# gardner-lab/syllable-detector-swift

Measured on AMD Instinct MI355X. Metric: audio frames/sec (256-pt STFT + 2-layer MLP), whole job, higher is better.
Workload: dtype f32 (I/O and accumulate; products as f16 hi/lo split x3 on MFMA)

## Files before the change

### syllable_detector_swift_amd/csrc/fused_plan.cpp

```cpp

#include <algorithm>
#include <cmath>
#include <cstdlib>
#include <cstring>

#include "fused_plan.hpp"

namespace sd {

namespace {

uint16_t to_half(float f)
{
    uint32_t x;
    std::memcpy(&x, &f, 4);
    const uint32_t sign = (x >> 16) & 0x8000u;
    const int32_t exp = (int32_t)((x >> 23) & 0xff) - 127 + 15;
    uint32_t man = x & 0x7fffffu;
    if (((x >> 23) & 0xff) == 0xff) return (uint16_t)(sign | 0x7c00u | (man ? 0x200u : 0));
    if (exp >= 31) return (uint16_t)(sign | 0x7c00u);
    if (exp <= 0) {
        if (exp < -10) return (uint16_t)sign;
        man |= 0x800000u;
        const int shift = 14 - exp;
        uint32_t h = man >> shift;
        const uint32_t rem = man & ((1u << shift) - 1), halfway = 1u << (shift - 1);
        if (rem > halfway || (rem == halfway && (h & 1))) h++;
        return (uint16_t)(sign | h);
    }
    uint32_t h = ((uint32_t)exp << 10) | (man >> 13);
    const uint32_t rem = man & 0x1fffu;
    if (rem > 0x1000u || (rem == 0x1000u && (h & 1))) h++;
    return (uint16_t)(sign | h);
}

float from_half(uint16_t h)
{
    const uint32_t sign = (uint32_t)(h & 0x8000u) << 16;
    const uint32_t exp = (h >> 10) & 0x1f, man = h & 0x3ffu;
// ... 148 lines not shown
        if (padp > W / 2) padp = 0;
#ifdef SYLDET_PLAN_NOPAD
        padp = 0;
#endif
        int chunk_bytes = 1024 + (padp ? 16 * (256 / padp) : 0);
        auto ring_chunks = [&](int waves) { return std::min(30, (160 * 1024 / waves - (row_bytes + 15) / 16 * 16) / chunk_bytes - 1); };
        auto fits = [&](int rc) { return rc >= (span + 255) / 256 + 1 && kFusedSTileFrames * hop <= rc * 256; };
        if (padp && !fits(ring_chunks(kFusedSBlock / 64))) {
            padp = 0;
            chunk_bytes = 1024;
        }
        const int s_waves = (!wide_band && (HQ == 1 || (HQ == 2 && fits(ring_chunks(kFusedSBlock / 64))))) ? kFusedSBlock / 64 : kFusedSBlock / 128;
        const int per_wave = 160 * 1024 / s_waves;
        const int RC = ring_chunks(s_waves);
        if (sym && H <= 16 && c.n_layers == 2 && fits(RC)) {
            d.s_ok = 1;
            d.s_waves = s_waves;
            d.s_padp = (padp && s_waves == kFusedSBlock / 64) ? padp : 0;
            d.s_perm = (hop / 4 + (d.s_padp ? hop / d.s_padp : 0)) % 2 == 1 ? 1 : 0;
#ifdef SYLDET_PLAN_NOPERM
            d.s_perm = (hop / 4) % 2 == 1 ? 1 : 0;
#endif
            d.s_ring_chunks = RC; d.s_pstride = PSs; d.s_tp = TP;
            d.s_lds_wave = per_wave;
            d.s_cs8 = 0;
            d.s_cs8_rc = 0;
            if (d.s_padp == 128 && hop == 128) {
                const int rc8 = std::min(16, (per_wave - (row_bytes + 15) / 16 * 16) / 1280);
                if (rc8 >= (span + 255) / 256 + 1) {
                    d.s_cs8 = 1;
                    d.s_cs8_rc = rc8;
                }
            }
            const int K2 = W / 64, c0 = W / 2;
            p.sfrag.assign((size_t)K2 * 2 * 2 * 2 * 64 * 8, 0);
            for (int ks = 0; ks < K2; ks++)
                for (int which = 0; which < 2; which++)
                    for (int m2 = 0; m2 < 2; m2++)
                        for (int l = 0; l < 64; l++)
                            for (int j = 0; j < 8; j++) {
                                const int r = 16 * m2 + (l & 15), m = 32 * ks + 8 * (l >> 4) + j;
                                double v = 0.0;
                                if (r < F) {
                                    const int k = g.f0 + r;
                                    const int kn = (int)(((int64_t)k * m) % N);
                                    const double ang = two_pi * (double)kn / (double)N;
                                    const double wm = 0.5 * ((double)win[(size_t)(c0 + m)] + (double)win[(size_t)(c0 - m)]);
                                    if (which == 0) {
                                        v = wm * std::cos(ang) * (m == 0 ? 0.5 : 1.0);
                                    } else if (m == 0) {
                                        const int kh = (int)(((int64_t)k * (W / 2)) % N);
                                        v = (double)win[0] * std::sin(two_pi * (double)kh / (double)N);
                                    } else {
                                        v = -wm * std::sin(ang);
                                    }
                                    if (which == 1 && k == 0) v = 0.0;
                                    v *= 8192.0;
                                }
                                uint16_t hi, lo;
                                split_half(v, hi, lo);
                                const size_t base = (((((size_t)ks * 2 + which) * 2 + m2) * 2) * 64 + l) * 8 + j;
                                p.sfrag[base] = hi;
                                p.sfrag[base + 64 * 8] = lo;
                            }
            p.slone.assign(64 * 8, 0.0f);
            for (int l = 0; l < 64; l++)
// ... 458 lines not shown
```

### syllable_detector_swift_amd/csrc/kernels.hpp

```cpp
#pragma once

#include <hip/hip_runtime.h>

#include <cstdint>

namespace sd {

constexpr int kMaxFns = 8;
constexpr int kMaxLayers = 8;

struct StftDesc {
    int N, W, M, logM;
    int hop, gap;
    int f0, F;
    int power_mode;
    const float *window;
    const float2 *tw;
    const float2 *sw;
    const int *row_of;
};

struct DevFn {
    int kind;
    int xoff, gain;
// ... 118 lines not shown
    int no_fold2;
    const uint4 *sfrag2;
    const float *swin2;
    const float *s2c;
    const uint4 *afrag_t2;
    const uint4 *afrag_w2;
    const uint4 *sfrag;
    const uint4 *afrag_w;
    const float *slone;
    const uint4 *dfrag;
    const uint4 *afrag;
    const uint4 *afrag_t;
    const int *koff;
    const float *bias0;
    const float *rvec;
    const float *w1, *b1;
    const float *out_params;
    const double *thresholds;
    float *spect_out;
    int spect_power;
    float guard_r;
    float guard_c;
    float guard_c_range;
    float guard_range_r;
    float guard_rel_r, guard_rel_c;
    int guard_se_abs_r, guard_se_abs_c;
    float guard_spect;
    int guard_se_abs_s;
    float guard_loud;
    FixList fix;
    int force_classic;
    int no_fold;
    int ko;
    unsigned long long *stamps;
};
struct FusedNet {
    const uint4 *afrag_t, *afrag_w, *afrag_t2, *afrag_w2;
    const float *bias0, *rvec, *w1, *b1, *out_params;
    const double *thresholds;
    float w_unscale, guard_r, guard_rel_r, guard_range_r, guard_loud;
    int guard_se_abs_r;
};
struct FusedMulti {
    const FusedNet *nets;
    const int *net_of;
    const int *row_of;
};

constexpr int kMlpxBlock = 512;
constexpr int kMlpxTile = 128;
struct MlpxDesc {
    int F, T, KB, H;
    int rule;
    int scaling;
    int col_stride;
    int p_stride;
    float w_unscale, b1, oa, og, ob;
    int lds_afrag, lds_colh, lds_coll, lds_p, lds_pq, lds_ss, lds_red, lds_total;
    const uint4 *afrag;
    const float *bias0, *w1;
    const double *thresholds;
};
constexpr int kBdftBlock = 512;
struct BdftDesc {
    int hop, kb0, f0;
    int R;
// ... 98 lines not shown
```

### syllable_detector_swift_amd/csrc/kernels_fused_s.hip

```cpp

#include "fused_common.hpp"

namespace sd {

namespace {

using namespace fused_dev;

constexpr int kTile = kFusedSTileFrames;

typedef __attribute__((address_space(3))) void lds_void;

__device__ __forceinline__ float rem_lo(float a, unsigned h)
{
    float r;
    asm("v_fma_mix_f32 %0, %1, 1.0, -%2 op_sel_hi:[0,0,1]" : "=v"(r) : "v"(a), "v"(h));
    return r;
}
__device__ __forceinline__ float rem_hi(float a, unsigned h)
{
    float r;
    asm("v_fma_mix_f32 %0, %1, 1.0, -%2 op_sel:[0,0,1] op_sel_hi:[0,0,1]" : "=v"(r) : "v"(a), "v"(h));
    return r;
}
__device__ __forceinline__ unsigned cvt_pk(float a, float b)
{
    unsigned r;
    asm("v_cvt_pk_f16_f32 %0, %1, %2" : "=v"(r) : "v"(a), "v"(b));
    return r;
}
__device__ __forceinline__ floatx4 s16x4(const int16_t *p)
{
    const uint2 v = *reinterpret_cast<const uint2 *>(p);
    constexpr float k = 1.0f / 32768.0f;
    return floatx4{(float)(int16_t)(v.x & 0xffffu) * k, (float)((int)v.x >> 16) * k, (float)(int16_t)(v.y & 0xffffu) * k,
                   (float)((int)v.y >> 16) * k};
}
__device__ __forceinline__ float s16x1(const int16_t *p) { return (float)p[0] * (1.0f / 32768.0f); }

__device__ __forceinline__ void split2(float a, float b, unsigned &hi, unsigned &lo)
{
    hi = cvt_pk(a, b);
    lo = cvt_pk(rem_lo(a, hi), rem_hi(b, hi));
}

template <int K2, bool GEN, int HQ, int NW, int PADP = 0, bool F2 = false, int NT = 1, bool SPECT = false, bool MN = false, bool S16 = false>
__global__ void __launch_bounds__(64 * NW, 1)
fused_s_kernel(const FusedDesc d, const float *__restrict__ samples, int64_t stride, int64_t s_eff, int64_t E,
               float *__restrict__ outputs, uint8_t *__restrict__ flags, const FusedNet *__restrict__ nets, const int *__restrict__ net_of,
               const int *__restrict__ row_of)
{
    static_assert(!(MN && SPECT), "the spectrogram instantiation runs no network");
    static_assert(!S16 || (K2 == 4 && F2 && PADP == 0 && NT == 1 && HQ == 1 && NW == 8 && !SPECT), "16-bit PCM: the twice-folded form on the plain ring");
    extern __shared__ __attribute__((aligned(16))) unsigned char smem[];
    const int tid = threadIdx.x;
    const int lane = tid & 63;
    const int wave = __builtin_amdgcn_readfirstlane(tid >> 6);
    const int n = lane & 15, g = lane >> 4;
    constexpr int kWaves = NW;
    const int c = blockIdx.y;
    const int T = d.T, H = d.H, hop = d.hop;
    constexpr int W = 64 * K2;
    const int n_out = GEN ? d.n_out : 1;
    const int64_t e_b = ((int64_t)blockIdx.x * kWaves + wave) * d.s_seg_evals;
    if (e_b >= E) return;
    const int64_t e_e = (e_b + d.s_seg_evals < E) ? e_b + d.s_seg_evals : E;
    const int seg_len = (int)(e_e - e_b);
    const int tiles = (seg_len + (T - 1) + kTile - 1) / kTile;
    const unsigned e_b32 = (unsigned)e_b;
    const FusedNet *nt = MN ? nets + __builtin_amdgcn_readfirstlane(net_of[c]) : nullptr;
#define SD_NET(f) (MN ? nt->f : d.f)

    const int fr = d.s_perm ? (n < 4 ? 2 * n : (n >= 12 ? 2 * (n - 8) : 2 * (n - 4) + 1)) : n;

    unsigned char *wbase = smem + (size_t)wave * d.s_lds_wave;
    const int RC = PADP == 1 ? d.s_cs8_rc : d.s_ring_chunks, R = RC * (S16 ? 512 : 256);
    constexpr bool CS8 = PADP == 1;
    static_assert(!CS8 || (F2 && HQ == 1 && NT == 1), "staggered chunks: the twice-folded form at hop 128");
    constexpr int kSub = PADP > 1 ? 256 / PADP : 1;
    constexpr int kChunkB = CS8 ? 1280 : 1024 + (PADP > 1 ? 16 * kSub : 0);
    auto sk = [](int i) { return PADP > 1 ? 4 * (i / (PADP > 1 ? PADP : 1)) : 0; };
    float *ring = reinterpret_cast<float *>(wbase);
    const int16_t *ring16 = reinterpret_cast<const int16_t *>(wbase);
    const int PS = d.s_pstride, TP = d.s_tp;
    float *rows = reinterpret_cast<float *>(wbase + (size_t)(RC + (CS8 ? 0 : 1)) * kChunkB);
    float *zquad = rows + (T - 1 + kTile) * PS;
    constexpr bool kTbl = HQ == 2 && NW == 8;
    float *gtab = zquad + 8 * HQ + 32 * g;
    {
        const int nz = ((T - 1 + kTile) * PS + 8 * HQ + 128) / 4;
        for (int i = lane; i < nz; i += 64) reinterpret_cast<floatx4 *>(rows)[i] = floatx4{0.f, 0.f, 0.f, 0.f};
    }

    constexpr int KB = F2 ? 1 : K2;
    half8 as_[KB][2][2], ad_[KB][2][2];
    if (!F2) {
#pragma unroll
        for (int ks = 0; ks < KB; ks++)
#pragma unroll
            for (int m = 0; m < 2; m++)
#pragma unroll
                for (int p = 0; p < 2; p++) {
                    as_[ks][m][p] = as_half8(reinterpret_cast<const uint32x4 *>(d.sfrag)[(((ks * 2 + 0) * 2 + m) * 2 + p) * 64 + lane]);
                    ad_[ks][m][p] = as_half8(reinterpret_cast<const uint32x4 *>(d.sfrag)[(((ks * 2 + 1) * 2 + m) * 2 + p) * 64 + lane]);
                }
    }
    half8 b2[F2 ? 2 : 1][F2 ? 4 * NT : 1][2];
    float w1c[F2 ? 16 : 1], w2c[F2 ? 16 : 1], ce[4 * NT], w192 = 0.0f;
#pragma unroll
// ... 38 lines not shown
    const int rc = MN ? bank_row(row_of, c) : c;
    const float *row = S16 ? reinterpret_cast<const float *>(reinterpret_cast<const int16_t *>(samples) + (int64_t)rc * stride)
                           : samples + (int64_t)rc * stride;
    const __amdgpu_buffer_rsrc_t in_rs = __builtin_amdgcn_make_buffer_rsrc(const_cast<float *>(row), 0, (int)(s_eff * (S16 ? 2 : 4)), 0x00020000);
    const __amdgpu_buffer_rsrc_t out_rs = __builtin_amdgcn_make_buffer_rsrc(
        outputs ? outputs + (int64_t)rc * E * n_out : nullptr, 0, outputs ? (int)(E * n_out * 4) : 0, 0x00020000);
    const __amdgpu_buffer_rsrc_t flg_rs = __builtin_amdgcn_make_buffer_rsrc(flags ? flags + (int64_t)rc * E : nullptr, 0, flags ? (int)E : 0, 0x00020000);
    const __amdgpu_buffer_rsrc_t spc_rs = __builtin_amdgcn_make_buffer_rsrc(
        SPECT ? d.spect_out + (int64_t)c * E * d.F : nullptr, 0, SPECT ? (int)(E * d.F * 4) : 0, 0x00020000);

    const unsigned org = (unsigned)((e_b * hop + d.gap) * (S16 ? 2 : 4));
    int cn = 0, slot = 0;
    auto issue_upto = [&](int last) {
        while (cn <= last) {
            const unsigned voff = org + (unsigned)cn * 1024u + (unsigned)lane * 16u;
            if (CS8) {
                const int pad = ((cn & 6) << 1) | (cn & 1);
                __builtin_amdgcn_raw_ptr_buffer_load_lds(in_rs, (lds_void *)(wbase + slot * kChunkB + 16 * pad), 16, voff, 0, 0, 2 );
            } else if (PADP == 0) {
                __builtin_amdgcn_raw_ptr_buffer_load_lds(in_rs, (lds_void *)(wbase + slot * 1024), 16, voff, 0, 0, 2 );
                if (slot == 0) __builtin_amdgcn_raw_ptr_buffer_load_lds(in_rs, (lds_void *)(wbase + RC * 1024), 16, voff, 0, 0, 2);
            } else {
#pragma unroll
                for (int k = 0; k < kSub; k++)
                    if (lane / (64 / kSub) == k) {
                        __builtin_amdgcn_raw_ptr_buffer_load_lds(in_rs, (lds_void *)(wbase + slot * kChunkB + 16 * k), 16, voff, 0, 0, 2);
                        if (slot == 0) __builtin_amdgcn_raw_ptr_buffer_load_lds(in_rs, (lds_void *)(wbase + RC * kChunkB + 16 * k), 16, voff, 0, 0, 2);
                    }
            }
            cn++;
            slot = slot + 1 == RC ? 0 : slot + 1;
        }
    };
    const int span = (kTile - 1) * hop + W;
    constexpr int kChunkLog = S16 ? 9 : 8;
    auto need = [&](int t) { return (kTile * hop * t + span - 1) >> kChunkLog; };
    auto allowed = [&](int t) { return RC - 1 + ((kTile * hop * t) >> kChunkLog); };

    unsigned fo = (unsigned)(hop * fr);
    unsigned sb1 = (unsigned)((fr >> 1) * kChunkB), sb2 = (unsigned)(((fr >> 1) + (fr & 1)) * kChunkB);
    const int jq1 = (fr >> 1) & 7, jq2 = ((fr >> 1) + (fr & 1)) & 7;
    const unsigned cb1 = (unsigned)(16 * (((jq1 & 6) << 1) | (jq1 & 1)) + ((fr & 1) ? 512 : 0));
    const unsigned cb2 = (unsigned)(16 * (((jq2 & 6) << 1) | (jq2 & 1)) + ((fr & 1) ? 0 : 512));
    float *prow = rows + (T - 1 + fr) * PS;
    const float *erow = rows + n * PS;
    const float *pv_p[3], *sv_p[3];
#pragma unroll
    for (int tt = 0; tt < 3; tt++) {
        const int t = g + 4 * tt;
        pv_p[tt] = t < T ? erow + t * PS + 4 * HQ * t : zquad;
        sv_p[tt] = t < T ? erow + t * PS + 4 * HQ * TP : zquad;
    }
    float *pt_p[3];
#pragma unroll
    for (int m = 0; m < 3; m++) pt_p[m] = 4 * m + g < TP ? prow + 4 * HQ * (4 * m + g) : zquad + 4 * HQ;

    const float c_b1 = GEN ? (g < n_out ? SD_NET(b1)[g] : 0.0f) : SD_NET(b1)[0];
    float lean_oa = 0.0f, lean_og = 1.0f, lean_ob = 0.0f;
    if (d.n_out_fns == 1) {
        const int o = (GEN && g < n_out) ? g : 0;
        lean_oa = SD_NET(out_params)[0]; lean_og = SD_NET(out_params)[1 + o]; lean_ob = SD_NET(out_params)[1 + n_out + o];
    }
    float b0g[HQ], w1g[HQ], w1o[4][HQ], rvg[HQ];
#pragma unroll
    for (int q = 0; q < HQ; q++) {
        const int u = 4 * q + g;
// ... 6 lines not shown
    if (kTbl && n == 0) {
#pragma unroll
        for (int q = 0; q < HQ; q++) {
            gtab[8 + q] = b0g[q];
            gtab[8 + HQ + q] = w1g[q];
            gtab[8 + 6 * HQ + q] = rvg[q];
#pragma unroll
            for (int o = 0; o < 4; o++) gtab[8 + 2 * HQ + o * HQ + q] = w1o[o][q];
        }
    }
    const bool multi = GEN && n_out > 1;
    const double thr_g = SD_NET(thresholds)[(GEN && g < n_out) ? g : 0];
    if (kTbl && n == 0) {
        gtab[22] = c_b1; gtab[23] = lean_oa; gtab[24] = lean_og; gtab[25] = lean_ob;
        *reinterpret_cast<double *>(gtab + 26) = thr_g;
    }
    const bool counts = !GEN || n_out == 1 ? true : (g < n_out && (g == 0 || d.rule == 1));
    const int tf0 = GEN ? d.tf0 : 0, tf1 = GEN ? d.tf1 : 2, norm = GEN ? d.norm : 1;
    const int scaling = GEN ? d.scaling : 0;
    const float klog = scaling == 1 ? 0.6931471805599453f : 6.020599913279624f;
    bool binv[8 * NT];
#pragma unroll
    for (int i = 0; i < 8 * NT; i++) {
        const int tau = i >> 3, ii = i & 7;
        binv[i] = (F2 ? 32 * tau + (ii < 4 ? 8 * g + d.s2_pe + 2 * ii : 8 * g + d.s2_po + 2 * (ii - 4)) : (ii < 4 ? 4 * g + ii : 16 + 4 * g + (ii - 4))) < d.F;
    }
    const float kmag = pow2f(-13 - d.col_shift);
    const bool guard_on = d.fix.counters != nullptr;
    const float guard_k = norm == 1 ? SD_NET(guard_r) : (norm == 0 ? SD_NET(guard_rel_r) : SD_NET(guard_range_r));
    const float mn_wu = MN ? nt->w_unscale : 0.0f, mn_loud = MN ? nt->guard_loud : 0.0f;
    const int mn_se_abs = MN ? nt->guard_se_abs_r : 0;
#undef SD_NET

    issue_upto(need(0) < allowed(0) ? need(0) : allowed(0));
    int se_ref = 0;

#ifdef SYLDET_S_STAMPS
    unsigned long long st_vm = 0, st_lg = 0;
    const unsigned long long st_begin = __builtin_amdgcn_s_memtime();
#define SD_STAMP(var, stmt) { asm volatile("s_waitcnt lgkmcnt(0)" ::: "memory"); const unsigned long long t0_ = __builtin_amdgcn_s_memtime(); stmt; \
                              const unsigned long long t1_ = __builtin_amdgcn_s_memtime(); var += t1_ - t0_; }
#else
#define SD_STAMP(var, stmt) { stmt; }
#endif
#ifndef SYLDET_S_NO_PREWAIT
    __builtin_amdgcn_s_waitcnt(0x0F70);
#endif
#if defined(SYLDET_S_SETPRIO_SECOND)
    if (wave >= kWaves / 2) __builtin_amdgcn_s_setprio(1);
#elif defined(SYLDET_S_SETPRIO_FIRST)
    if (wave < kWaves / 2) __builtin_amdgcn_s_setprio(1);
#endif
    for (int t = 0; t < tiles; t++) {
        SD_STAMP(st_vm, if (t == 0) asm volatile("s_waitcnt vmcnt(0)" ::: "memory"); else if (SPECT) asm volatile("s_waitcnt vmcnt(5)" ::: "memory");
                        else asm volatile("s_waitcnt vmcnt(2)" ::: "memory"));
        const float *f1 = reinterpret_cast<const float *>(wbase + sb1 + cb1);
        const float *f2 = reinterpret_cast<const float *>(wbase + sb2 + cb2);
        const float *fp = CS8 ? f1 : ring + fo + sk((int)fo);

        floatx4 P1[2][2], P3[2][2], P2[2][2], P4[2][2];
        float P2w[2], P4w[2], x64 = 0.0f, x192 = 0.0f;
        if (F2) {
#pragma unroll
            for (int ks = 0; ks < 2; ks++) {
                if (CS8) {
                    const float *a1 = f1 + 32 * ks + 8 * g, *a2 = f2 + 32 * ks + 8 * g;
                    const float *b1 = f1 + 120 - 32 * ks - 8 * g, *b3 = f2 + 120 - 32 * ks - 8 * g;
// ... 8 lines not shown
                    P4[ks][1] = *reinterpret_cast<const floatx4 *>(b3 + 4);
                    P4w[ks] = b3[8];
                    continue;
                }
                if (S16) {
                    const int16_t *a = ring16 + fo + 32 * ks + 8 * g, *b = ring16 + fo + 120 - 32 * ks - 8 * g;
                    P1[ks][0] = s16x4(a);
                    P1[ks][1] = s16x4(a + 4);
                    P3[ks][0] = s16x4(a + 128);
                    P3[ks][1] = s16x4(a + 132);
                    P2[ks][0] = s16x4(b);
                    P2[ks][1] = s16x4(b + 4);
                    P2w[ks] = s16x1(b + 8);
                    P4[ks][0] = s16x4(b + 128);
                    P4[ks][1] = s16x4(b + 132);
                    P4w[ks] = s16x1(b + 136);
                    continue;
                }
                const float *a = fp + 32 * ks + 8 * g, *b = fp + 120 - 32 * ks - 8 * g;
                P1[ks][0] = *reinterpret_cast<const floatx4 *>(a);
                P1[ks][1] = *reinterpret_cast<const floatx4 *>(a + 4);
                P3[ks][0] = *reinterpret_cast<const floatx4 *>(a + 128 + sk(128));
                P3[ks][1] = *reinterpret_cast<const floatx4 *>(a + 132 + sk(128));
                P2[ks][0] = *reinterpret_cast<const floatx4 *>(b + sk(64));
                P2[ks][1] = *reinterpret_cast<const floatx4 *>(b + 4 + sk(64));
                P2w[ks] = (PADP && ks == 0) ? b[8 + (g == 0 ? sk(128) : sk(64))] : b[8 + sk(64)];
                P4[ks][0] = *reinterpret_cast<const floatx4 *>(b + 128 + sk(192));
                P4[ks][1] = *reinterpret_cast<const floatx4 *>(b + 132 + sk(192));
                P4w[ks] = b[136 + sk(192)];
            }
            x64 = S16 ? s16x1(ring16 + fo + 64) : (CS8 ? f1[64] : fp[64 + sk(64)]);
            x192 = S16 ? s16x1(ring16 + fo + 192) : (CS8 ? f2[64] : fp[192 + sk(192)]);
            SD_STAMP(st_lg, asm volatile("s_waitcnt lgkmcnt(0)" ::: "memory"));
            if (t + 1 < tiles) issue_upto(need(t + 1));
        }
        float amax;
#ifdef SYLDET_S_NOMAX
        amax = 1.0f;
#else
        {
            float m0 = 0.0f, m1 = 0.0f;
            if (F2) {
#pragma unroll
                for (int ks = 0; ks < 2; ks++)
#pragma unroll
                    for (int h = 0; h < 2; h++) {
                        m0 = absmax3(m0, P1[ks][h][0], P1[ks][h][1]);
                        m1 = absmax3(m1, P1[ks][h][2], P1[ks][h][3]);
                        m0 = absmax3(m0, P3[ks][h][0], P3[ks][h][1]);
                        m1 = absmax3(m1, P3[ks][h][2], P3[ks][h][3]);
                        m0 = absmax3(m0, P2[ks][h][0], P2[ks][h][1]);
                        m1 = absmax3(m1, P2[ks][h][2], P2[ks][h][3]);
                        m0 = absmax3(m0, P4[ks][h][0], P4[ks][h][1]);
                        m1 = absmax3(m1, P4[ks][h][2], P4[ks][h][3]);
                    }
                m0 = absmax3(m0, P2w[0], P2w[1]);
                m1 = absmax3(m1, g == 0 ? 0.0f : P4w[0], P4w[1]);
                m0 = absmax3(m0, x64, x192);
            } else {
                const floatx4 *q0 = reinterpret_cast<const floatx4 *>(fp + (W / 4) * g + sk((W / 4) * g));
#pragma unroll
                for (int q = 0; q < W / 16; q++) {
                    const floatx4 v = q0[q];
                    m0 = absmax3(m0, v[0], v[1]);
                    m1 = absmax3(m1, v[2], v[3]);
                }
            }
// ... 238 lines not shown
#pragma unroll
                for (int i = 0; i < 8 * NT; i++) {
                    mn = binv[i] ? fminf(mn, cval[i]) : mn;
                    mx = binv[i] ? fmaxf(mx, cval[i]) : mx;
                }
                auto r = __builtin_amdgcn_permlane16_swap(__float_as_uint(mn), __float_as_uint(mn), false, false);
                mn = fminf(__uint_as_float(r[0]), __uint_as_float(r[1]));
                r = __builtin_amdgcn_permlane32_swap(__float_as_uint(mn), __float_as_uint(mn), false, false);
                mn = fminf(__uint_as_float(r[0]), __uint_as_float(r[1]));
                r = __builtin_amdgcn_permlane16_swap(__float_as_uint(mx), __float_as_uint(mx), false, false);
                mx = fmaxf(__uint_as_float(r[0]), __uint_as_float(r[1]));
                r = __builtin_amdgcn_permlane32_swap(__float_as_uint(mx), __float_as_uint(mx), false, false);
                mx = fmaxf(__uint_as_float(r[0]), __uint_as_float(r[1]));
                st0 = mn * pow2f(dsc);
                st1 = mx * pow2f(dsc);
            } else if (GEN && norm == 3) {
                float sm = 0.0f;
#pragma unroll
                for (int i = 0; i < 8 * NT; i++) sm += binv[i] ? cval[i] : 0.0f;
                sm = xor32_sum(xor16_sum(sm));
                const float mean = sm / (float)d.F;
                float m2 = 0.0f;
#pragma unroll
                for (int i = 0; i < 8 * NT; i++) {
                    const float dl = cval[i] - mean;
                    m2 = binv[i] ? fmaf(dl, dl, m2) : m2;
                }
                m2 = xor32_sum(xor16_sum(m2));
                st0 = mean * pow2f(dsc);
                st1 = m2 * pow2f(2 * dsc);
            }
            if (GEN && norm == 0) st1 = st0;
            const float fw = far ? INFINITY : ((fst == 1 || (GEN && scaling != 0)) ? 0.0f : pow2f(2 * dsc));
            if (g == 0) *reinterpret_cast<floatx4 *>(prow + 4 * HQ * TP) = floatx4{st0, fw, st1, 0.0f};
        }

        floatx4 zp[HQ];
        float ssp, fwp, st1p = 0.0f;
        float sq0[3];
        const int nq = (T - 1) * PS / 4;
        floatx4 cy0 = {0.f, 0.f, 0.f, 0.f}, cy1 = cy0, cy2 = cy0;
        if (HQ == 1) {
            const floatx4 *src = reinterpret_cast<const floatx4 *>(rows + kTile * PS);
            cy0 = src[lane < nq ? lane : 0];
            cy1 = src[lane + 64 < nq ? lane + 64 : 0];
            if (nq > 128) cy2 = src[lane + 128 < nq ? lane + 128 : 0];
        }
        {
            floatx4 pv[3][HQ];
#pragma unroll
            for (int tt = 0; tt < 3; tt++)
#pragma unroll
                for (int q = 0; q < HQ; q++) pv[tt][q] = *reinterpret_cast<const floatx4 *>(pv_p[tt] + 4 * q);
            const floatx4 s0 = *reinterpret_cast<const floatx4 *>(sv_p[0]), s1 = *reinterpret_cast<const floatx4 *>(sv_p[1]),
                          s2 = *reinterpret_cast<const floatx4 *>(sv_p[2]);
            sq0[0] = s0[0]; sq0[1] = s1[0]; sq0[2] = s2[0];
#pragma unroll
            for (int q = 0; q < HQ; q++) zp[q] = pv[0][q] + pv[1][q] + pv[2][q];
            if (GEN && (norm == 0 || norm == 2)) {
                ssp = fminf(fminf(g < T ? s0[0] : INFINITY, g + 4 < T ? s1[0] : INFINITY), g + 8 < T ? s2[0] : INFINITY);
                st1p = norm == 0 ? s0[2] + s1[2] + s2[2]
                                 : fmaxf(fmaxf(g < T ? s0[2] : -INFINITY, g + 4 < T ? s1[2] : -INFINITY), g + 8 < T ? s2[2] : -INFINITY);
            } else {
                ssp = s0[0] + s1[0] + s2[0];
                st1p = s0[2] + s1[2] + s2[2];
            }
            fwp = fmaxf(fmaxf(s0[1], s1[1]), s2[1]);
// ... 127 lines not shown
            }
        }
        const int er = kTile * t - (T - 1) + n;
        const bool vld = er >= 0 && er < seg_len;
        {
            const bool st = vld && g == 0, sto = vld && g < n_out;
            const unsigned off = e_b32 + (unsigned)er;
            __builtin_amdgcn_raw_buffer_store_b32(__float_as_uint(yv), out_rs, sto ? (off * (unsigned)n_out + (unsigned)g) * 4u : 0xFFFFFFFFu, 0, 0);
            __builtin_amdgcn_raw_buffer_store_b8((unsigned char)(hit ? 1 : 0), flg_rs, st ? off : 0xFFFFFFFFu, 0, 0);
        }
        if (guard_on) {
            bool bad = vld && !(fww == 0.0f) && !(gstat >= guard_k * ((GEN && norm >= 2) ? sqrtf(fww) : fww));
            if (GEN && norm == 0 && fww != INFINITY && fww != 0.0f) {
                const int lg = (int)((__float_as_uint(fww) >> 23) & 0xffu) - 127;
                if (se_ref - lg / 2 >= (MN ? mn_se_abs : d.guard_se_abs_r)) bad = false;
            }
            if (GEN && norm == 0 && scaling == 0 && vld) {
                const int ush2 = 2 * (d.col_shift - se_ref);
                const float u2 = st1w * pow2f(ush2 < -120 ? -120 : (ush2 > 120 ? 120 : ush2));
                if (u2 * (MN ? mn_loud : d.guard_loud) > 1.0f) bad = true;
            }
            if (__builtin_amdgcn_ballot_w64(bad) != 0ull) {
                const int er0 = kTile * t - (T - 1);
                const int lo = er0 < 0 ? 0 : er0, hi = er0 + kTile < seg_len ? er0 + kTile : seg_len;
                if (lane == 0 && hi > lo) {
                    const unsigned sl = atomicAdd(d.fix.counters, 1u);
                    if (sl < d.fix.capacity) d.fix.items[sl] = FixItem{c, e_b32 + (unsigned)lo, hi - lo, 0};
                    else d.fix.counters[3] = 1u;
                }
            }
        }
        {
            floatx4 *dst = reinterpret_cast<floatx4 *>(rows);
            if (HQ == 1) {
                if (lane < nq) dst[lane] = cy0;
                if (lane + 64 < nq) dst[lane + 64] = cy1;
                if (nq > 128 && lane + 128 < nq) dst[lane + 128] = cy2;
            } else {
                const floatx4 *src = reinterpret_cast<const floatx4 *>(rows + kTile * PS);
                for (int i = lane; i < nq; i += 64) dst[i] = src[i];
            }
        }
        fo += (unsigned)(kTile * hop);
        fo = fo >= (unsigned)R ? fo - (unsigned)R : fo;
        if (CS8) {
            sb1 += 8u * kChunkB; sb1 = sb1 >= (unsigned)(RC * kChunkB) ? sb1 - (unsigned)(RC * kChunkB) : sb1;
            sb2 += 8u * kChunkB; sb2 = sb2 >= (unsigned)(RC * kChunkB) ? sb2 - (unsigned)(RC * kChunkB) : sb2;
        }
    }
#ifdef SYLDET_S_STAMPS
    if (d.stamps && lane == 0) {
        atomicAdd(d.stamps + 0, __builtin_amdgcn_s_memtime() - st_begin);
        atomicAdd(d.stamps + 1, st_vm);
        atomicAdd(d.stamps + 2, st_lg);
        atomicAdd(d.stamps + 3, (unsigned long long)tiles);
        atomicAdd(d.stamps + 4, 1ull);
    }
#endif
#undef SD_STAMP
}

template <int K2, bool GEN, int HQ, int NW, int PADP = 0, bool F2 = false, int NT = 1, bool SPECT = false, bool MN = false, bool S16 = false>
hipError_t launch_one(const FusedDesc &d, const float *samples, int64_t stride, int C, int64_t s_eff, int64_t E,
                      float *outputs, uint8_t *flags, hipStream_t stream, const FusedMulti *mn = nullptr)
{
    if constexpr (!SPECT && !MN)
        if (mn) return launch_one<K2, GEN, HQ, NW, PADP, F2, NT, false, true, S16>(d, samples, stride, C, s_eff, E, outputs, flags, stream, mn);
    if (fused_note_form(2, K2, GEN, HQ, NW, PADP, F2, NT, SPECT, MN, S16)) return hipSuccess;
    auto kern = fused_s_kernel<K2, GEN, HQ, NW, PADP, F2, NT, SPECT, MN, S16>;
    constexpr int kWaves = NW;
#ifdef SYLDET_S_ONEWAVE
    const int lds = kWaves == 4 ? 100 * 1024 : d.s_lds_wave * kWaves;
#else
    const int lds = d.s_lds_wave * kWaves;
#endif
    hipError_t st = hipFuncSetAttribute((const void *)kern, hipFuncAttributeMaxDynamicSharedMemorySize, lds);
    if (st != hipSuccess) return st;
    const int64_t segs = (E + d.s_seg_evals - 1) / d.s_seg_evals;
    dim3 grid((unsigned)((segs + kWaves - 1) / kWaves), (unsigned)C);
    const FusedNet *nets = MN ? mn->nets : nullptr;
    const int *net_of = MN ? mn->net_of : nullptr;
    const int *row_of = MN ? mn->row_of : nullptr;
    hipLaunchKernelGGL(kern, grid, dim3(64 * kWaves), (size_t)lds, stream, d, samples, stride, s_eff, E, outputs, flags, nets, net_of, row_of);
    return hipGetLastError();
}

}

bool fused_s_has_stamps()
{
#ifdef SYLDET_S_STAMPS
    return true;
#else
    return false;
#endif
}

bool fused_s_applicable(const FusedDesc &d)
{
    const bool cls = d.norm >= 0 && d.norm <= 3 && d.n_layers == 2 && d.n_out >= 1 && d.n_out <= 4 && d.H <= 16 && d.n_out_fns <= 1;
    if (d.F > 32 && !(d.s2_ok && d.s2_nt == 2 && !d.no_fold2)) return false;
    return d.s_ok && d.T <= 12 && cls;
// ... 97 lines not shown
```

### syllable_detector_swift_amd/csrc/syldet_api.cpp

```cpp

#include <hip/hip_runtime.h>

#include <algorithm>
#include <atomic>
#include <cmath>
#include <cstdio>
#include <cstdlib>
#include <cstring>
#include <deque>
#include <map>
#include <memory>
#include <mutex>
#include <new>
#include <string>
#include <vector>

#include "fused_plan.hpp"
#include "kernels.hpp"
#include "sample_ring.hpp"
#include "syldet_internal.hpp"

using namespace sd;

namespace {
// ... 54 lines not shown
        ptr = nullptr;
        cap = 0;
    }
};

}

struct syldet {
    OwnedConfig cfg;
    syldet_geometry_t geom{};
    int channels = 0;
    int device = 0;
    int engine = SYLDET_ENGINE_GENERIC;
    int engine_asked = SYLDET_ENGINE_AUTO;

    struct Switches {
        bool fused_classic = false;
        bool no_fft1k = false;
        bool wide_no_front = false;
        bool wide_wg16 = false;
        bool wide_stagger = true;
        bool wide_dma_builtin = false;
        bool wide_tiles4 = false;
        bool wide_m32 = false;
        bool wide_tanh_poly = false;
        bool wide_shape32 = false;
        bool no_bdft = false;
        bool no_stft_lanes = false;
        bool no_guard = false;
        bool no_mlpx = false;
        bool fused_nofold = false;
        bool fused_pad128 = false;
        bool fused_nofold2 = false;
        bool fused_stamps = false;
        int fused_ko = 0;
        long long host_chunk = 0;
        void read()
        {
            host_chunk = std::getenv("SYLDET_HOST_CHUNK_BYTES") ? std::atoll(std::getenv("SYLDET_HOST_CHUNK_BYTES")) : 0;
            fused_classic = std::getenv("SYLDET_FUSED_CLASSIC") != nullptr;
            no_fft1k = std::getenv("SYLDET_NO_FFT1K") != nullptr;
            no_bdft = std::getenv("SYLDET_NO_BDFT") != nullptr;
            wide_shape32 = std::getenv("SYLDET_WIDE_SHAPE32") != nullptr;
            wide_wg16 = std::getenv("SYLDET_WIDE_WG16") != nullptr;
            wide_stagger = std::getenv("SYLDET_WIDE_NOSTAGGER") == nullptr;
            wide_dma_builtin = std::getenv("SYLDET_WIDE_DMA_BUILTIN") != nullptr;
            wide_tiles4 = std::getenv("SYLDET_WIDE_T4") != nullptr;
            wide_tanh_poly = std::getenv("SYLDET_WIDE_TANH_POLY") != nullptr;
            wide_m32 = std::getenv("SYLDET_WIDE_M32") != nullptr;
            wide_no_front = std::getenv("SYLDET_WIDE_NO_FRONT") != nullptr;
            no_stft_lanes = std::getenv("SYLDET_NO_STFT_LANES") != nullptr;
            no_guard = std::getenv("SYLDET_NO_GUARD") != nullptr;
            no_mlpx = std::getenv("SYLDET_NO_MLPX") != nullptr;
            fused_nofold = std::getenv("SYLDET_FUSED_NOFOLD") != nullptr;
            fused_nofold2 = std::getenv("SYLDET_FUSED_NOFOLD2") != nullptr;
            fused_pad128 = std::getenv("SYLDET_FUSED_PAD128") != nullptr;
            fused_stamps = std::getenv("SYLDET_FUSED_STAMPS") != nullptr;
            fused_ko = std::getenv("SYLDET_FUSED_KO") ? std::atoi(std::getenv("SYLDET_FUSED_KO")) : 0;
        }
    } sw;

    DeviceBuffer d_window, d_tw, d_sw, d_params, d_thr;
    StftDesc stft{};
    NetDesc net{};

    DeviceBuffer d_columns;

    FusedPlan fused;
    DeviceBuffer d_stamps;
    DeviceBuffer d_fix;
    DeviceBuffer d_ctab;
    FixDesc fixd{};
    bool has_fix = false;
    DeviceBuffer d_fused;
    DeviceBuffer d_stage_in, d_stage_out, d_stage_flags, d_stage_idx, d_stage_cnt;
    DeviceBuffer d_planar;
    DeviceBuffer d_widen;

    FusedPlan dft;
    DeviceBuffer d_dft;
    bool has_dft = false;

    MlpxPlan mlpx;
    DeviceBuffer d_mlpx;
    BdftPlan bdft;
    DeviceBuffer d_bdft;

    WideDesc wide{};
// ... 489 lines not shown
int timed_fixup(syldet *hc, hipStream_t stream, FixList list, F launch)
{
    syldet *h = hc->root ? hc->root : hc;
    if (h->profiling && !h->prof_calls.empty() && list.counters) {
        if (h->prof_items_n < h->prof_depth) {
            SYLDET_HIP(hipDeviceSynchronize());
            if (h->prof_items) (void)hipHostFree(h->prof_items);
            h->prof_items = nullptr; h->prof_items_dev = nullptr; h->prof_items_n = 0;
            SYLDET_HIP(hipHostMalloc(reinterpret_cast<void **>(&h->prof_items), 2 * sizeof(unsigned) * (size_t)h->prof_depth, hipHostMallocMapped));
            SYLDET_HIP(hipHostGetDevicePointer(reinterpret_cast<void **>(&h->prof_items_dev), h->prof_items, 0));
            h->prof_items_n = h->prof_depth;
            for (int i = 0; i < 2 * h->prof_items_n; i++) h->prof_items[i] = 0u;
        }
        syldet::ProfCall &pc = h->prof_calls[(size_t)h->prof_cur()];
        pc.fix = true;
        pc.fix_stream = stream;
        list.host_count = h->prof_items_dev + 2 * h->prof_cur();
    }
    SYLDET_HIP(launch(list));
    return SYLDET_OK;
}

bool dft_route_for(const syldet *h, int64_t J, int C, bool for_network, const int *row_of, float *d_columns, FusedDesc &d, bool &fold)
{
    const bool log_input = for_network && h->cfg.view.scaling != SYLDET_SCALING_LINEAR;
    const bool level_input = for_network && !normalised_chain(h->cfg.view) && h->engine != SYLDET_ENGINE_WIDE_BF16 && h->engine_asked == SYLDET_ENGINE_AUTO;
    if (!(h->has_dft && !log_input && !level_input && !row_of && (uint64_t)J * (uint64_t)h->geom.bins * 4u < 0xFFFFFFF0ull)) return false;
    d = h->dft.desc;
    fused_segmentation(d, J, C);
    d.spect_out = d_columns;
    d.stamps = nullptr;
    d.ko = 0;
    d.no_fold2 = h->sw.fused_nofold2 ? 1 : 0;
    d.no_cs8 = h->sw.fused_pad128 ? 1 : 0;
    fold = !h->sw.fused_nofold && fused_s_spectrogram_applicable(d) && ((J - 1) * (int64_t)d.hop + d.gap + d.W) * 4 < 0x7fffffffll;
    return fold || d.classic_ok;
}

int stft_on_stream(syldet *h, const float *d_samples, int64_t stride, int C, int64_t J, float *d_columns, hipStream_t stream,
                   bool for_network = true, const int *row_of = nullptr)
{
    FusedDesc d{};
    bool fold = false;
    if (dft_route_for(h, J, C, for_network, row_of, d_columns, d, fold)) {
        if (int st = prepare_fix(h, C, J, (J + d.seg_evals - 1) / d.seg_evals + (d.s_seg_evals > 0 ? (J + d.s_seg_evals - 1) / d.s_seg_evals : 0), stream, d.fix)) return st;
        if (fold) {
            KernelTimer t(h, stream, "fused_s_kernel (spectrogram)");
            SYLDET_HIP(launch_fused_s_spectrogram(d, d_samples, stride, C, J, stream));
        } else {
            KernelTimer t(h, stream, "fused_kernel (spectrogram)");
            SYLDET_HIP(launch_fused_spectrogram(d, d_samples, stride, C, J, stream));
        }
        note_fused_launch(h);
        return timed_fixup(h, stream, d.fix, [&](const FixList &l) { return launch_fixup(h->fixd, h->net, d_samples, stride, J, 0, nullptr, nullptr, d_columns, l, stream); });
    }
    StftDesc sd = h->stft;
    sd.row_of = row_of;
    if (!h->sw.no_stft_lanes && stft_lanes_applicable(sd, d_samples, stride)) {
        KernelTimer t(h, stream, "stft_lanes_kernel");
        SYLDET_HIP(launch_stft_lanes(sd, d_samples, stride, C, J, d_columns, stream));
        return SYLDET_OK;
    }
    KernelTimer t(h, stream, "stft_generic_kernel");
    SYLDET_HIP(launch_stft_generic(sd, d_samples, stride, C, J, d_columns, stream));
    return SYLDET_OK;
}

struct Samples {
    const void *p = nullptr;
    bool s16 = false;
    Samples(const float *f) : p(f) {}
    Samples(const void *q, bool pcm16) : p(q), s16(pcm16) {}
};

bool fused_route_for(const syldet *h, int64_t J, int64_t E, int C, FusedDesc &d)
{
    bool fused_route = h->engine == SYLDET_ENGINE_FUSED && (uint64_t)E * (uint64_t)h->geom.outputs * 4u < 0xFFFFFFF0ull;
    if (fused_route) {
        d = h->fused.desc;
        fused_segmentation(d, E, C);
        d.stamps = nullptr;
        d.fix = FixList{nullptr, nullptr, 0};
        d.ko = h->sw.fused_ko;
        d.force_classic = h->sw.fused_classic ? 1 : 0;
        d.no_fold = h->sw.fused_nofold ? 1 : 0;
        d.no_fold2 = h->sw.fused_nofold2 ? 1 : 0;
        d.no_cs8 = h->sw.fused_pad128 ? 1 : 0;
        const int choice = fused_choice(d, J);
        const bool runnable = choice != 0 || d.classic_ok;
        const bool in_contract = ((h->cfg.view.scaling == SYLDET_SCALING_LINEAR && normalised_chain(h->cfg.view)) || choice == 2 || h->engine_asked == SYLDET_ENGINE_FUSED);
        if (!runnable || !in_contract) fused_route = false;
        if ((h->n_nets > 1 || h->fnets) && (choice != 2 || h->sw.fused_stamps)) fused_route = false;
    }
    return fused_route;
}

bool takes_native_s16(const syldet *h, Samples x, int64_t S, int64_t stride, int C)
{
    const int64_t J = count_frames(h, S), E = count_evals(h, S);
    FusedDesc d{};
    if (E <= 0 || !fused_route_for(h, J, E, C, d)) return false;
    return fused_choice(d, J) == 2 && !h->sw.fused_stamps && fused_s_native_s16(d) && (reinterpret_cast<uintptr_t>(x.p) & 3) == 0 &&
           (stride & 1) == 0 && (d.gap & 1) == 0;
}

int widen_s16(syldet *h, Samples &x, int64_t S, int64_t &stride, int C, hipStream_t stream)
{
    syldet *owner = h->root ? h->root : h;
    const int64_t ws = (S + 3) & ~(int64_t)3;
    if (int st = owner->d_widen.reserve((size_t)C * (size_t)ws * sizeof(float))) return st;
    {
        KernelTimer t(h, stream, "widen_s16_kernel");
        SYLDET_HIP(launch_widen_s16((const int16_t *)x.p, stride, S, C, (float *)owner->d_widen.ptr, ws, stream));
    }
    x = Samples((const float *)owner->d_widen.ptr);
    stride = ws;
    return SYLDET_OK;
}

// ... 130 lines not shown
    }
    if (int st = stft_on_stream(h, d_samples, stride, C, J, (float *)h->d_columns.ptr, stream, true, d_row_of)) return st;
    if (h->mlpx.ok && (uint64_t)E * 4u < 0xFFFFFFF0ull) {
        KernelTimer t(h, stream, "mlp_mfma_kernel");
        SYLDET_HIP(launch_mlpx(h->mlpx.desc, (const float *)h->d_columns.ptr, C, J, E, d_outputs, d_flags, stream));
        return SYLDET_OK;
    }
    {
        KernelTimer t(h, stream, "mlp_generic_kernel");
        SYLDET_HIP(launch_mlp_generic(net, h->geom.bins, (const float *)h->d_columns.ptr, C, J, E, d_outputs,
                                      d_flags, stream));
    }
    return SYLDET_OK;
}

int check_batch_args(const syldet *h, const void *samples, int64_t S, int64_t stride)
{
    if (!h) return fail(SYLDET_ERR_INVALID_ARGUMENT, "NULL handle");
    if (S < 0) return fail(SYLDET_ERR_INVALID_ARGUMENT, "n_samples must be >= 0");
    if (!samples && S > 0) return fail(SYLDET_ERR_INVALID_ARGUMENT, "NULL samples");
    if (h->channels > 1 && stride < S) return fail(SYLDET_ERR_INVALID_ARGUMENT, "channel_stride must be >= n_samples");
    return SYLDET_OK;
}

bool takes_fold(const syldet_config_t &c, const syldet_geometry_t &g, const syldet::Switches &sw, bool &fused_ok)
{
    fused_ok = false;
    FusedPlan plan;
    if (!make_fused_plan(c, g, plan) || !fused_s_applicable(plan.desc)) return false;
    FusedDesc d = plan.desc;
    d.force_classic = sw.fused_classic ? 1 : 0;
    d.no_fold = sw.fused_nofold ? 1 : 0;
    d.no_fold2 = sw.fused_nofold2 ? 1 : 0;
    d.no_cs8 = sw.fused_pad128 ? 1 : 0;
    d.ko = sw.fused_ko;
    d.stamps = nullptr;
    fused_ok = fused_choice(d, 1) == 2;
    return fused_ok && (c.scaling == SYLDET_SCALING_LINEAR || d.norm == 1);
}

int upload_fold_nets(syldet *h, const std::vector<std::unique_ptr<OwnedConfig>> &cfgs)
{
    const size_t K = cfgs.size();
    std::vector<FusedPlan> plans(K);
    for (size_t k = 0; k < K; k++) {
        if (!make_fused_plan(cfgs[k]->view, h->geom, plans[k]))
            return fail(SYLDET_ERR_UNSUPPORTED, "fold kernel plan failed for network " + std::to_string(k) + ": " + plans[k].reason);
        const FusedDesc &a = plans[0].desc, &b = plans[k].desc;
        if (a.s_ok != b.s_ok || a.s2_ok != b.s2_ok || a.s2_nt != b.s2_nt || a.s_padp != b.s_padp || a.s_cs8 != b.s_cs8 ||
            a.s_waves != b.s_waves || a.s_lds_wave != b.s_lds_wave || a.col_shift != b.col_shift || a.H != b.H || a.norm != b.norm)
            return fail(SYLDET_ERR_UNSUPPORTED, "network " + std::to_string(k) + " gives the fold kernel another shape");
    }
    auto pad = [](size_t b) { return (b + 255) / 256 * 256; };
    const int n_thr = h->cfg.view.n_thresholds;
    const FusedPlan &p0 = plans[0];
    const size_t sz[10] = {p0.afrag_t.size() * 2, p0.afrag_w.size() * 2, p0.afrag_t2.size() * 2, p0.afrag_w2.size() * 2, p0.bias0.size() * 4,
                           p0.rvec.size() * 4, p0.w1.size() * 4, p0.b1.size() * 4, p0.out_params.size() * 4, (size_t)n_thr * 8};
    size_t off[10], stride = 0;
    for (int i = 0; i < 10; i++) {
        off[i] = stride;
        stride += pad(std::max<size_t>(sz[i], 16));
    }
    std::vector<unsigned char> blob(stride * K + pad(K * sizeof(FusedNet)), 0);
    for (size_t k = 0; k < K; k++) {
        const FusedPlan &p = plans[k];
        const void *src[10] = {p.afrag_t.data(), p.afrag_w.data(), p.afrag_t2.data(), p.afrag_w2.data(), p.bias0.data(),
// ... 1549 lines not shown
```

Baseline: 9.348 billion.

## Add compile-time hop-132 ring schedule with unrolled per-phase chunk issue

Adds a specialised kernel instantiation for hop 132 and window 256. It uses a fixed 11-slot LDS ring whose chunk issue pattern repeats every four tiles and is unrolled at compile time per phase, with one mirrored slot so a frame never wraps. This replaces the runtime issue_upto bookkeeping and the ring-wrap arithmetic. It also drops lane guards on a few LDS stores by clamping addresses instead. The path only triggers when the configured hop is 132, and it adds another template instantiation and an environment switch to turn it off.

Result: faster. 9.474 billion, median of 6 (+1.4%).

```diff
diff --git a/syllable_detector_swift_amd/csrc/fused_plan.cpp b/syllable_detector_swift_amd/csrc/fused_plan.cpp
--- a/syllable_detector_swift_amd/csrc/fused_plan.cpp
+++ b/syllable_detector_swift_amd/csrc/fused_plan.cpp
@@ -5,6 +5,7 @@
 #include <cstring>
 
 #include "fused_plan.hpp"
+#include "hopk_schedule.hpp"
 
 namespace sd {
 
@@ -219,6 +220,9 @@
                     d.s_cs8_rc = rc8;
                 }
             }
+            d.s_hopk_rc = 0;
+            if (hop == hopk::kHop && W == hopk::kWindow && HQ == 1 && d.s_padp == 0 && s_waves == kFusedSBlock / 64 && RC >= hopk::kRing && fits(hopk::kRing))
+                d.s_hopk_rc = hopk::kRing;
             const int K2 = W / 64, c0 = W / 2;
             p.sfrag.assign((size_t)K2 * 2 * 2 * 2 * 64 * 8, 0);
             for (int ks = 0; ks < K2; ks++)
diff --git a/syllable_detector_swift_amd/csrc/hopk_schedule.hpp b/syllable_detector_swift_amd/csrc/hopk_schedule.hpp
--- /dev/null
+++ b/syllable_detector_swift_amd/csrc/hopk_schedule.hpp
@@ -0,0 +1,34 @@
+#pragma once
+
+namespace sd {
+namespace hopk {
+
+constexpr int kHop = 132;
+constexpr int kTileFrames = 16;
+constexpr int kWindow = 256;
+constexpr int kChunk = 256;
+constexpr int kRing = 11;
+constexpr int kPeriod = 4;
+constexpr int kPeriodChunks = 33;
+constexpr int kTileAdvance = kTileFrames * kHop;
+constexpr int kSpan = (kTileFrames - 1) * kHop + kWindow;
+constexpr int kRingFloats = kRing * kChunk;
+
+static_assert(kPeriod * kTileAdvance == kPeriodChunks * kChunk, "the period is a whole number of chunks");
+static_assert(kPeriodChunks % kRing == 0, "the slot pattern closes with the period");
+static_assert(kTileAdvance <= kRingFloats && kHop % 4 == 0, "a lane's frame offset stays inside the ring, on a quad");
+
+constexpr int first_chunk(int ph) { return (kTileAdvance * ph) / kChunk; }
+constexpr int last_chunk(int ph) { return (kTileAdvance * ph + kSpan - 1) / kChunk; }
+constexpr int issue_first(int ph) { return last_chunk(ph) + 1; }
+constexpr int issue_last(int ph) { return last_chunk(ph + 1); }
+constexpr int slot_of(int q) { return q % kRing; }
+constexpr bool mirrored(int q) { return q % kRing == 0; }
+constexpr int frame0_offset(int ph) { return (kTileAdvance * ph) % kRingFloats; }
+
+constexpr bool phase_fits(int ph) { return issue_last(ph) - kRing < first_chunk(ph + 1) && last_chunk(ph) - first_chunk(ph) < kRing; }
+static_assert(phase_fits(0) && phase_fits(1) && phase_fits(2) && phase_fits(3), "eleven slots hold a tile's span and the next tile's chunks");
+static_assert(last_chunk(kPeriod) == last_chunk(0) + kPeriodChunks && first_chunk(kPeriod) == kPeriodChunks, "phase 4 is phase 0, one period on");
+
+}
+}
diff --git a/syllable_detector_swift_amd/csrc/kernels.hpp b/syllable_detector_swift_amd/csrc/kernels.hpp
--- a/syllable_detector_swift_amd/csrc/kernels.hpp
+++ b/syllable_detector_swift_amd/csrc/kernels.hpp
@@ -174,6 +174,7 @@
     int force_classic;
     int no_fold;
     int ko;
+    int s_hopk_rc;
     unsigned long long *stamps;
 };
 struct FusedNet {
diff --git a/syllable_detector_swift_amd/csrc/kernels_fused_s.hip b/syllable_detector_swift_amd/csrc/kernels_fused_s.hip
--- a/syllable_detector_swift_amd/csrc/kernels_fused_s.hip
+++ b/syllable_detector_swift_amd/csrc/kernels_fused_s.hip
@@ -1,5 +1,6 @@
 
 #include "fused_common.hpp"
+#include "hopk_schedule.hpp"
 
 namespace sd {
 
@@ -44,7 +45,18 @@
     lo = cvt_pk(rem_lo(a, hi), rem_hi(b, hi));
 }
 
-template <int K2, bool GEN, int HQ, int NW, int PADP = 0, bool F2 = false, int NT = 1, bool SPECT = false, bool MN = false, bool S16 = false>
+template <int QF, int QL>
+__device__ __forceinline__ void hopk_issue(__amdgpu_buffer_rsrc_t in_rs, unsigned char *wbase, unsigned pv)
+{
+#pragma unroll
+    for (int q = QF; q <= QL; q++) {
+        const unsigned voff = pv + (unsigned)q * 1024u;
+        __builtin_amdgcn_raw_ptr_buffer_load_lds(in_rs, (lds_void *)(wbase + hopk::slot_of(q) * 1024), 16, voff, 0, 0, 2 );
+        if (hopk::mirrored(q)) __builtin_amdgcn_raw_ptr_buffer_load_lds(in_rs, (lds_void *)(wbase + hopk::kRing * 1024), 16, voff, 0, 0, 2);
+    }
+}
+
+template <int K2, bool GEN, int HQ, int NW, int PADP = 0, bool F2 = false, int NT = 1, bool SPECT = false, bool MN = false, bool S16 = false, int HOP = 0>
 __global__ void __launch_bounds__(64 * NW, 1)
 fused_s_kernel(const FusedDesc d, const float *__restrict__ samples, int64_t stride, int64_t s_eff, int64_t E,
                float *__restrict__ outputs, uint8_t *__restrict__ flags, const FusedNet *__restrict__ nets, const int *__restrict__ net_of,
@@ -52,6 +64,8 @@
 {
     static_assert(!(MN && SPECT), "the spectrogram instantiation runs no network");
     static_assert(!S16 || (K2 == 4 && F2 && PADP == 0 && NT == 1 && HQ == 1 && NW == 8 && !SPECT), "16-bit PCM: the twice-folded form on the plain ring");
+    static_assert(HOP == 0 || (HOP == hopk::kHop && K2 == 4 && F2 && PADP == 0 && NT == 1 && HQ == 1 && NW == 8 && !SPECT && !S16 && kFusedSTileFrames == hopk::kTileFrames),
+                  "a compile-time hop: 132, the twice-folded form on the plain fp32 ring, one quad of units on eight waves");
     extern __shared__ __attribute__((aligned(16))) unsigned char smem[];
     const int tid = threadIdx.x;
     const int lane = tid & 63;
@@ -59,7 +73,7 @@
     const int n = lane & 15, g = lane >> 4;
     constexpr int kWaves = NW;
     const int c = blockIdx.y;
-    const int T = d.T, H = d.H, hop = d.hop;
+    const int T = d.T, H = d.H, hop = HOP ? HOP : d.hop;
     constexpr int W = 64 * K2;
     const int n_out = GEN ? d.n_out : 1;
     const int64_t e_b = ((int64_t)blockIdx.x * kWaves + wave) * d.s_seg_evals;
@@ -74,7 +88,7 @@
     const int fr = d.s_perm ? (n < 4 ? 2 * n : (n >= 12 ? 2 * (n - 8) : 2 * (n - 4) + 1)) : n;
 
     unsigned char *wbase = smem + (size_t)wave * d.s_lds_wave;
-    const int RC = PADP == 1 ? d.s_cs8_rc : d.s_ring_chunks, R = RC * (S16 ? 512 : 256);
+    const int RC = HOP ? hopk::kRing : (PADP == 1 ? d.s_cs8_rc : d.s_ring_chunks), R = RC * (S16 ? 512 : 256);
     constexpr bool CS8 = PADP == 1;
     static_assert(!CS8 || (F2 && HQ == 1 && NT == 1), "staggered chunks: the twice-folded form at hop 128");
     constexpr int kSub = PADP > 1 ? 256 / PADP : 1;
@@ -179,6 +193,9 @@
             slot = slot + 1 == RC ? 0 : slot + 1;
         }
     };
+    unsigned pv = 0;
+    int ph = 0;
+    if constexpr (HOP != 0) pv = org + (unsigned)lane * 16u;
     const int span = (kTile - 1) * hop + W;
     constexpr int kChunkLog = S16 ? 9 : 8;
     auto need = [&](int t) { return (kTile * hop * t + span - 1) >> kChunkLog; };
@@ -251,7 +268,8 @@
     const int mn_se_abs = MN ? nt->guard_se_abs_r : 0;
 #undef SD_NET
 
-    issue_upto(need(0) < allowed(0) ? need(0) : allowed(0));
+    if constexpr (HOP != 0) hopk_issue<0, hopk::last_chunk(0)>(in_rs, wbase, pv);
+    else issue_upto(need(0) < allowed(0) ? need(0) : allowed(0));
     int se_ref = 0;
 
 #ifdef SYLDET_S_STAMPS
@@ -326,7 +344,18 @@
             x64 = S16 ? s16x1(ring16 + fo + 64) : (CS8 ? f1[64] : fp[64 + sk(64)]);
             x192 = S16 ? s16x1(ring16 + fo + 192) : (CS8 ? f2[64] : fp[192 + sk(192)]);
             SD_STAMP(st_lg, asm volatile("s_waitcnt lgkmcnt(0)" ::: "memory"));
-            if (t + 1 < tiles) issue_upto(need(t + 1));
+            if constexpr (HOP != 0) {
+                static_assert(hopk::kPeriod == 4, "one case a phase");
+                if (t + 1 < tiles) {
+                    if (ph == 0) hopk_issue<hopk::issue_first(0), hopk::issue_last(0)>(in_rs, wbase, pv);
+                    else if (ph == 1) hopk_issue<hopk::issue_first(1), hopk::issue_last(1)>(in_rs, wbase, pv);
+                    else if (ph == 2) hopk_issue<hopk::issue_first(2), hopk::issue_last(2)>(in_rs, wbase, pv);
+                    else {
+                        hopk_issue<hopk::issue_first(3), hopk::issue_last(3)>(in_rs, wbase, pv);
+                        pv += (unsigned)(hopk::kPeriodChunks * 1024);
+                    }
+                }
+            } else if (t + 1 < tiles) issue_upto(need(t + 1));
         }
         float amax;
 #ifdef SYLDET_S_NOMAX
@@ -631,7 +660,8 @@
             }
             if (GEN && norm == 0) st1 = st0;
             const float fw = far ? INFINITY : ((fst == 1 || (GEN && scaling != 0)) ? 0.0f : pow2f(2 * dsc));
-            if (g == 0) *reinterpret_cast<floatx4 *>(prow + 4 * HQ * TP) = floatx4{st0, fw, st1, 0.0f};
+            if constexpr (HOP != 0) *reinterpret_cast<floatx4 *>(prow + 4 * HQ * TP) = floatx4{st0, fw, st1, 0.0f};
+            else if (g == 0) *reinterpret_cast<floatx4 *>(prow + 4 * HQ * TP) = floatx4{st0, fw, st1, 0.0f};
         }
 
         floatx4 zp[HQ];
@@ -825,7 +855,11 @@
         }
         {
             floatx4 *dst = reinterpret_cast<floatx4 *>(rows);
-            if (HQ == 1) {
+            if constexpr (HOP != 0) {
+                dst[lane < nq ? lane : 0] = cy0;
+                dst[lane + 64 < nq ? lane + 64 : 0] = cy1;
+                if (nq > 128) dst[lane + 128 < nq ? lane + 128 : 0] = cy2;
+            } else if (HQ == 1) {
                 if (lane < nq) dst[lane] = cy0;
                 if (lane + 64 < nq) dst[lane + 64] = cy1;
                 if (nq > 128 && lane + 128 < nq) dst[lane + 128] = cy2;
@@ -836,6 +870,7 @@
         }
         fo += (unsigned)(kTile * hop);
         fo = fo >= (unsigned)R ? fo - (unsigned)R : fo;
+        if constexpr (HOP != 0) ph = (ph + 1) & (hopk::kPeriod - 1);
         if (CS8) {
             sb1 += 8u * kChunkB; sb1 = sb1 >= (unsigned)(RC * kChunkB) ? sb1 - (unsigned)(RC * kChunkB) : sb1;
             sb2 += 8u * kChunkB; sb2 = sb2 >= (unsigned)(RC * kChunkB) ? sb2 - (unsigned)(RC * kChunkB) : sb2;
@@ -861,6 +896,13 @@
         if (mn) return launch_one<K2, GEN, HQ, NW, PADP, F2, NT, false, true, S16>(d, samples, stride, C, s_eff, E, outputs, flags, stream, mn);
     if (fused_note_form(2, K2, GEN, HQ, NW, PADP, F2, NT, SPECT, MN, S16)) return hipSuccess;
     auto kern = fused_s_kernel<K2, GEN, HQ, NW, PADP, F2, NT, SPECT, MN, S16>;
+    if constexpr (K2 == 4 && HQ == 1 && NW == 8 && PADP == 0 && F2 && NT == 1 && !SPECT && !S16) {
+        if (d.hop == hopk::kHop && d.s_hopk_rc != 0) {
+            if (d.s_hopk_rc != hopk::kRing || (d.s_hopk_rc + 1) * 1024 + ((d.T - 1 + kTile) * d.s_pstride + 8 * HQ + 128) * 4 > d.s_lds_wave)
+                return hipErrorInvalidValue;
+            kern = fused_s_kernel<K2, GEN, HQ, NW, PADP, F2, NT, SPECT, MN, S16, hopk::kHop>;
+        }
+    }
     constexpr int kWaves = NW;
 #ifdef SYLDET_S_ONEWAVE
     const int lds = kWaves == 4 ? 100 * 1024 : d.s_lds_wave * kWaves;
diff --git a/syllable_detector_swift_amd/csrc/syldet_api.cpp b/syllable_detector_swift_amd/csrc/syldet_api.cpp
--- a/syllable_detector_swift_amd/csrc/syldet_api.cpp
+++ b/syllable_detector_swift_amd/csrc/syldet_api.cpp
@@ -110,6 +110,7 @@
         bool fused_nofold = false;
         bool fused_pad128 = false;
         bool fused_nofold2 = false;
+        bool fused_nohopk = false;
         bool fused_stamps = false;
         int fused_ko = 0;
         long long host_chunk = 0;
@@ -132,6 +133,7 @@
             no_mlpx = std::getenv("SYLDET_NO_MLPX") != nullptr;
             fused_nofold = std::getenv("SYLDET_FUSED_NOFOLD") != nullptr;
             fused_nofold2 = std::getenv("SYLDET_FUSED_NOFOLD2") != nullptr;
+            fused_nohopk = std::getenv("SYLDET_FUSED_HOPK") != nullptr && std::atoi(std::getenv("SYLDET_FUSED_HOPK")) == 0;
             fused_pad128 = std::getenv("SYLDET_FUSED_PAD128") != nullptr;
             fused_stamps = std::getenv("SYLDET_FUSED_STAMPS") != nullptr;
             fused_ko = std::getenv("SYLDET_FUSED_KO") ? std::atoi(std::getenv("SYLDET_FUSED_KO")) : 0;
@@ -687,6 +689,7 @@
     d.stamps = nullptr;
     d.ko = 0;
     d.no_fold2 = h->sw.fused_nofold2 ? 1 : 0;
+    if (h->sw.fused_nohopk) d.s_hopk_rc = 0;
     d.no_cs8 = h->sw.fused_pad128 ? 1 : 0;
     fold = !h->sw.fused_nofold && fused_s_spectrogram_applicable(d) && ((J - 1) * (int64_t)d.hop + d.gap + d.W) * 4 < 0x7fffffffll;
     return fold || d.classic_ok;
@@ -740,6 +743,7 @@
         d.force_classic = h->sw.fused_classic ? 1 : 0;
         d.no_fold = h->sw.fused_nofold ? 1 : 0;
         d.no_fold2 = h->sw.fused_nofold2 ? 1 : 0;
+        if (h->sw.fused_nohopk) d.s_hopk_rc = 0;
         d.no_cs8 = h->sw.fused_pad128 ? 1 : 0;
         const int choice = fused_choice(d, J);
         const bool runnable = choice != 0 || d.classic_ok;
@@ -936,6 +940,7 @@
     d.force_classic = sw.fused_classic ? 1 : 0;
     d.no_fold = sw.fused_nofold ? 1 : 0;
     d.no_fold2 = sw.fused_nofold2 ? 1 : 0;
+    if (sw.fused_nohopk) d.s_hopk_rc = 0;
     d.no_cs8 = sw.fused_pad128 ? 1 : 0;
     d.ko = sw.fused_ko;
     d.stamps = nullptr;
```
